# MingruiYuan/SpoofSV

Hardware: AMD Instinct MI355X
Metric: mel-frames/sec (Text2Mel+SSRN train) (higher is better)
Workload: dtype f32 (conv GEMMs: fp32 operands scaled by a power of two and split into fp16 hi+lo = 22 significand bits, three exact fp16 MFMAs per product, fp32 accumulate: ~2^-22 per product, gradients within 3e-6 of float64 = the exact-fp32 path's level); 1 GPU; train_text2mel + train_ssrn (train/ordinary.py step: fwd, l1+bin-div+guided-att losses, bwd, Adam), batch 32 utterances/GPU, N=186, T=325, 80 mel -> 513x1300 linear, hidden 256, random-init; global_batch=32, parallelism=dp1, launch=hipGraph replay, ddp=none

## Files before the change

spoofsv_amd/csrc/ssv_common.h:

```cpp
#pragma once
#include <hip/hip_runtime.h>
#include <stdint.h>
#include <stddef.h>
#include "../../include/ssv_hip.h"

int ssv_fail(int code, const char* fmt, ...);
#define SSV_BAD_SHAPE (-1)
#define SSV_UNSUPPORTED (-2)
#define SSV_CHECK(cond, code, ...) do { if (!(cond)) return ssv_fail((code), __VA_ARGS__); } while (0)
#define SSV_TRY(expr) do { int _e = (expr); if (_e) return _e; } while (0)
int ssv_check_launch(const char* what);

typedef __attribute__((ext_vector_type(4))) float f32x4;

struct GemmNN {
  const float* A = nullptr; long sab = 0, sam = 0, sac = 0, saj = 0;
  const float* X = nullptr; long sxb = 0, sxc = 0, sxn = 1; int Lx = 0;
  float* C = nullptr; long scb = 0, scm = 0, scn = 1;
  const float* bias = nullptr;
  const float* bias_b = nullptr; long sbb = 0;
  const float* R = nullptr; long srb = 0, srm = 0, srn = 1;
  int M = 0, N = 0, Kc = 0, KT = 1, B = 1;
  int shift[3] = {0, 0, 0};
  float alpha = 1.f;
};
int ssv_launch_gemm_nn(const GemmNN& g, hipStream_t st);

struct GemmNT {
  const float* A = nullptr; long sab = 0, sam = 0, sat = 1; int La = 0;
  const float* X = nullptr; long sxb = 0, sxc = 0, sxn = 1; int Lx = 0;
  float* C = nullptr; long scz = 0, scm = 0, scc = 1, scj = 0;
  int M = 0, Nc = 0, KT = 1, B = 1, Z = 1, bstep = 1;
  int shift[3] = {0, 0, 0};
  const ssv_wgrad_job* jobs = nullptr; int njobs = 0;
  int max_shift = -1;
  int f16 = 0; const float* a_amax = nullptr; int a_namax = 0; const float* x_amax = nullptr; int x_namax = 0;
};
int ssv_launch_gemm_nt(const GemmNT& g, hipStream_t st);

struct GemmNNB {
  const unsigned short* Ahi = nullptr; const unsigned short* Alo = nullptr; int Kpad = 0;
  const float* X = nullptr; long sxb = 0, sxc = 0; int Lx = 0;
  float* C = nullptr; long scb = 0, scm = 0;
  const float* bias = nullptr;
  const float* bias_b = nullptr; long sbb = 0;
  const float* R = nullptr; long srb = 0, srm = 0;
  int M = 0, N = 0, Kc = 0, KT = 1, B = 1;
  int shift[3] = {0, 0, 0};
  int sxn = 1, scn = 1;
  int row_pair = 0; float* c_amax = nullptr; int c_namax = 0;
  unsigned short* hs_planes = nullptr; long hs_plane_bytes = 0; int hs_npad = 0;
  int hs_keep_h = 1;
  int ksplit = 1; long scz = 0; int skip_rows = 0;
  const unsigned short* x0_planes = nullptr; const float* x0_amax = nullptr; int xsplit0 = 0;
  int perm_h = 0, epi = 0, first = 0;
  float* cstate = nullptr;
  float* lstm_out = nullptr; int lstm_s = 0, lstm_lo = 0, lstm_D = 0, xsplit = 0; long sab = 0;
  const unsigned short* A0hi = nullptr; const unsigned short* A0lo = nullptr;
  float* gates_out = nullptr;
  int f16 = 0; const float* a_inv = nullptr; const float* x_amax = nullptr; int x_namax = 0; long x_amax_bs = 0;
  float* colstats = nullptr;
  const float* xrow_w = nullptr; long xrow_sk = 0;
};
int ssv_launch_gemm_nn_bf3(const GemmNNB& g, hipStream_t st);
int ssv_launch_gemm_pwln(const GemmNNB& g, const float* gamma, const float* beta, float* y, long ybs, float* stats, float* y_amax, int namax, int act,
                         hipStream_t st);
int ssv_launch_gemm_nt_bf3(const GemmNT& g, hipStream_t st);
int ssv_launch_gemm_nt3r(const GemmNT& g, dim3 grid, int mtiles, int tchunks, int ring_ms, hipStream_t st);
struct PwLnBw {
  const float* dy; long dy_bs; const float* pre; const float* stats; const float* gamma; const float* beta;
  float* dpre; float* part; int part_rows; int part_q; float* amax; int namax;
  const unsigned short* Ahi; const unsigned short* Alo; const float* a_inv;
  float* dx; long dx_bs; const float* xrow_w; long xrow_sk;
  int M, Cin, L, act;
};
bool ssv_pwln_bwd_fused_ok(int B, int Cin, int Cout, int L);
int ssv_launch_pwln_bwd(const PwLnBw& q, int B, int f16, hipStream_t st);
bool ssv_nt_bf3_xrow(int KT, int M, int Nc);
bool ssv_nt_bf3_fits(const GemmNT& g);
int ssv_launch_pack_split(const float* w, void* hi, void* lo, int M, int K, int Kpad, int KT, long sm, long sk, long sj, int perm_h, hipStream_t st,
                          int nch_total = 0, int ch_off = 0);
int ssv_launch_pack_split_f16(const float* w, long w_elems, void* hi, void* lo, int M, int K, int Kpad, int KT, long sm, long sk, long sj, float* aux, hipStream_t st);
int ssv_launch_pack_split_f16_list(const float* w, void* hi, void* lo, int M, int K, int Kpad, int KT, long sm, long sk, long sj, int perm_h,
                                   const float* list, int nlist, float* inv_out, hipStream_t st, int nch_total = 0, int ch_off = 0);
#define SSV_F16_AUX_FLOATS 128
#define SSV_AMAX_FALLBACK 64
int ssv_launch_absmax(const float* x, long x_bs, int B, long n, float* out, int npb, hipStream_t st);
int ssv_nt_bf3_tiles(int KT, int M, int Nc);
void ssv_nt_bf3_tile(int KT, int M, int Nc, int* wm, int* ntc);
int ssv_nt_bf3_wg_per_cu(int KT, int wm, int ntc);
int ssv_precision();
enum { SSV_T_NT_FORCE, SSV_T_NNB_FORCE, SSV_T_LN_GROUPS, SSV_T_LN_PERSIST, SSV_T_LSTM_MERGE, SSV_T_PWLN_BWD, SSV_T_COUNT };
const char* ssv_tuning(int knob);
int ssv_pack_job_blocks(const ssv_pack_job& j);
int ssv_launch_pack_multi(const ssv_pack_job* jobs_dev, int njobs, int nblocks, float* amax_ws, hipStream_t st);
#define SSV_PACK_AMAX_PER_WEIGHT 32

int ssv_launch_reduce_slabs(const float* slabs, float* out, long n, int Z, long slab_stride, hipStream_t st);
int ssv_launch_reduce_slabs_perm(const float* slabs, float* out, int M, int Nc, int KT, int Z, hipStream_t st);
int ssv_launch_reduce_pair(const float* slabs, float* out, int M, int Nc, int KT, int Z, const float* part, float* pout, int n2, int nblk, hipStream_t st);
int ssv_launch_reduce_pair_multi(const ssv_wgrad_job* jobs, int njobs, const float* slabs, int M, int Nc, int KT, int Z, int n2, int nblk, hipStream_t st);
int ssv_launch_pack_wt(const float* w, float* wt, int Cout, int Cin, int KT, hipStream_t st);
int ssv_launch_fill(float* p, float v, long n, hipStream_t st);
int ssv_launch_linear_len1_fwd(const float* x, long x_bs, const float* w, const float* bias, const float* bias_b, long sbb, float* y, long y_bs,
                               int B, int K, int M, hipStream_t st);
int ssv_launch_linear_len1_wgrad(const float* dy, long dy_bs, const float* x, long x_bs, float* dw, int B, int K, int M, hipStream_t st);

static inline int ssv_cdiv(long a, long b) { return (int)((a + b - 1) / b); }
bool ssv_shape_log_on();
void ssv_shape_log(const char* kernel, dim3 grid, dim3 block, double flops, double bytes, const char* note);
__host__ __device__ static inline int ssv_amax_rows_(int L) { return 4 * ((L + 63) / 64); }

__device__ __forceinline__ unsigned ssv_xcd_order(unsigned lin, unsigned total) {
  const unsigned xcd = lin & 7u, idx = lin >> 3, q = total >> 3, r = total & 7u;
  return xcd * q + (xcd < r ? xcd : r) + idx;
}

__device__ __forceinline__ void ssv_pow2_scale(float amax, float& scale, float& inv) {
  int E = (int)((__float_as_uint(amax) >> 23) & 0xffu);
  E = min(max(E, 15), 254);
  scale = __uint_as_float((unsigned)(268 - E) << 23);
  inv = __uint_as_float((unsigned)(E - 14) << 23);
}
typedef unsigned ssv_u32x4g __attribute__((vector_size(16)));
__device__ __forceinline__ __amdgpu_buffer_rsrc_t ssv_buf(const void* base) {
  return __builtin_amdgcn_make_buffer_rsrc(const_cast<void*>(base), 0, -1, 0x00020000);
}
__device__ __forceinline__ float ssv_buf_f32(__amdgpu_buffer_rsrc_t r, unsigned voff, unsigned soff) {
  return __builtin_bit_cast(float, __builtin_amdgcn_raw_buffer_load_b32(r, (int)voff, (int)soff, 0));
}
__device__ __forceinline__ uint4 ssv_buf_u4(__amdgpu_buffer_rsrc_t r, unsigned voff, unsigned soff) {
  return __builtin_bit_cast(uint4, __builtin_amdgcn_raw_buffer_load_b128(r, (int)voff, (int)soff, 0));
}
template <class T> __device__ __forceinline__ T* ssv_global(T* p) {
  return (T*)(__attribute__((address_space(1))) T*)p;
}
__device__ __forceinline__ float ssv_uniform(float v) { return __builtin_bit_cast(float, __builtin_amdgcn_readfirstlane(__builtin_bit_cast(int, v))); }
template <int NW>
__device__ __forceinline__ float ssv_wg_max(float v, float* sm) {
#pragma unroll
  for (int o = 1; o < 64; o <<= 1) v = fmaxf(v, __shfl_xor(v, o));
  if ((threadIdx.x & 63) == 0) sm[threadIdx.x >> 6] = v;
  __syncthreads();
  float r = sm[0];
#pragma unroll
  for (int i = 1; i < NW; ++i) r = fmaxf(r, sm[i]);
  return r;
}
template <int CTRL> __device__ __forceinline__ float ssv_dpp_mov(float v);
template <int CTRL>
__device__ __forceinline__ float ssv_dpp_max(float v) { return fmaxf(v, ssv_dpp_mov<CTRL>(v)); }
__device__ __forceinline__ float ssv_wave_list_max(const float* __restrict__ p, int n) {
  float v = 0.f;
  for (int i = threadIdx.x & 63; i < n; i += 64) v = fmaxf(v, p[i]);
  v = ssv_dpp_max<0xB1>(v);
  v = ssv_dpp_max<0x4E>(v);
  v = ssv_dpp_max<0x141>(v);
  v = ssv_dpp_max<0x140>(v);
  const int b = __builtin_bit_cast(int, v);
  const float r0 = __builtin_bit_cast(float, __builtin_amdgcn_readlane(b, 0)), r1 = __builtin_bit_cast(float, __builtin_amdgcn_readlane(b, 16));
  const float r2 = __builtin_bit_cast(float, __builtin_amdgcn_readlane(b, 32)), r3 = __builtin_bit_cast(float, __builtin_amdgcn_readlane(b, 48));
  return fmaxf(fmaxf(r0, r1), fmaxf(r2, r3));
}
template <int NW>
__device__ __forceinline__ float ssv_list_max(const float* __restrict__ p, int n, float* sm) {
  float v = 0.f;
  for (int i = threadIdx.x; i < n; i += 64 * NW) v = fmaxf(v, p[i]);
  return ssv_wg_max<NW>(v, sm);
}

template <int CTRL>
__device__ __forceinline__ float ssv_dpp_mov(float v) {
  return __builtin_bit_cast(float, __builtin_amdgcn_update_dpp(0, __builtin_bit_cast(int, v), CTRL, 0xf, 0xf, true));
}
__device__ __forceinline__ float ssv_row16_sum(float v) {
  v += ssv_dpp_mov<0xB1>(v);
  v += ssv_dpp_mov<0x4E>(v);
  v += ssv_dpp_mov<0x141>(v);
  v += ssv_dpp_mov<0x140>(v);
  return v;
}
__device__ __forceinline__ float ssv_wave_sum(float v) {
  v = ssv_row16_sum(v);
  v += __shfl_xor(v, 16);
  v += __shfl_xor(v, 32);
  return v;
}
```

spoofsv_amd/csrc/wgrad_nt.hip:

```cpp
#include "bf3_common.h"

#ifdef SSV_NT_STAMP
__device__ unsigned long long ssv_nt_stamps[64];
__device__ unsigned long long ssv_nt_wg[4096 * 4];
extern "C" int ssv_debug_nt_wg(unsigned long long* out) { return (int)hipMemcpyFromSymbol(out, HIP_SYMBOL(ssv_nt_wg), sizeof(ssv_nt_wg)); }
#define NT_WG(k, v) do { const unsigned w_ = blockIdx.z * gridDim.x + blockIdx.x; if (threadIdx.x == 0 && w_ < 4096u) ssv_nt_wg[w_ * 4 + (k)] = (v); } while (0)
#define NT_STAMP(k) do { if (stamp_on && (unsigned)(stamp_s - 24) < 8u) ssv_nt_stamps[(stamp_s - 24) * 8 + (k)] = __builtin_readcyclecounter(); } while (0)
extern "C" int ssv_debug_nt_stamps(unsigned long long* out) { return (int)hipMemcpyFromSymbol(out, HIP_SYMBOL(ssv_nt_stamps), sizeof(ssv_nt_stamps)); }
#else
#define NT_STAMP(k) do {} while (0)
#define NT_WG(k, v) do {} while (0)
#endif
constexpr int NT_FD = 1;
template <int KT, int WM, int NTC, int F16, int XR = 0, int WV = 4>
__global__ __launch_bounds__(64 * WV, WV == 4 ? 2 : 1) void gemm_nt_bf3_kernel(const GemmNT p, const int mtiles) {
  constexpr int NTH = 64 * WV;
  constexpr int KB = 64, KG = KB / 8, KS = KB / 32;
  constexpr int NCH = 16 * NTC;
  constexpr int X_SLOTS = KG * NCH;
  constexpr int NX = X_SLOTS / NTH;
  static_assert(X_SLOTS % NTH == 0, "tile slots must be a multiple of the workgroup size");
  __shared__ uint4 lds[2][2 * X_SLOTS];
  __shared__ float amax_sm[2 * WV];

  const int tid = threadIdx.x, lane = tid & 63, wave = tid >> 6;
  NT_WG(0, __builtin_amdgcn_s_memrealtime()); NT_WG(2, __builtin_readcyclecounter());
  const unsigned wg = ssv_xcd_order(blockIdx.x + gridDim.x * blockIdx.z, gridDim.x * gridDim.z);
  const int bxx = (int)(wg % gridDim.x);
  int z = (int)(wg / gridDim.x);
  const float* __restrict__ Ap = p.A;
  const float* __restrict__ Xp = p.X;
  float* __restrict__ Cp = p.C;
  int shj[3] = {p.shift[0], p.shift[1], p.shift[2]};
  const float* __restrict__ a_amax = p.a_amax;
  const float* __restrict__ x_amax = p.x_amax;
  int a_namax = p.a_namax, x_namax = p.x_namax;
  if (p.jobs) {
    const int job = z / p.Z;
    z -= job * p.Z;
    const ssv_wgrad_job* __restrict__ jb = p.jobs + job;
    Ap = ssv_global(jb->dy); Xp = ssv_global(jb->x); Cp = p.C + (long)job * p.Z * p.scz;
    shj[0] = jb->shift[0]; shj[1] = jb->shift[1]; shj[2] = jb->shift[2];
    a_amax = ssv_global(jb->dy_amax); x_amax = ssv_global(jb->x_amax); a_namax = jb->dy_namax; x_namax = jb->x_namax;
  }
  float as = 1.f, xs = 1.f, us = 1.f;
  auto scales = [&]() {
    if constexpr (F16) {
      float sa, sx, ia, ix;
      ssv_pow2_scale(ssv_list_max<WV>(a_amax, a_namax, amax_sm), sa, ia);
      ssv_pow2_scale(ssv_list_max<WV>(x_amax, x_namax, amax_sm + WV), sx, ix);
      as = ssv_uniform(sa); xs = ssv_uniform(sx);
      us = ssv_uniform(ia * ix);
    }
  };
  const int ctiles_ = (int)gridDim.x / mtiles;
  const bool ct_fast = gridDim.x > 64u;
  const int mt = ct_fast ? bxx / ctiles_ : bxx % mtiles, ct = ct_fast ? bxx % ctiles_ : bxx / mtiles;
  const int m0 = mt * 16 * WV * WM, c0 = ct * NCH;
  const int tchunks = (p.La + KB - 1) / KB;
  const int kq = lane >> 4, nq = lane & 15;

  f32x4 acc[WM][KT][NTC];
#pragma unroll
  for (int i = 0; i < WM; ++i)
#pragma unroll
    for (int j = 0; j < KT; ++j)
#pragma unroll
      for (int q = 0; q < NTC; ++q) acc[i][j][q] = (f32x4){0.f, 0.f, 0.f, 0.f};

  float rx[NX][8];
  int mx[NX];
  static_assert(!XR || (KT == 1 && WV == 4 && (256 % KG) == 0), "extra row: k = 1; a thread's slots share their k-group");
  const bool xr_on = XR && mt == 0;
  float xacc[XR ? NX : 1];
  uint4 xra[XR ? 2 : 1];
#pragma unroll
  for (int r = 0; r < (XR ? NX : 1); ++r) xacc[r] = 0.f;
  uint4 AH[2][WM][KS], AL[2][WM][KS];

  const __amdgpu_buffer_rsrc_t rsA = __builtin_amdgcn_make_buffer_rsrc(const_cast<float*>(Ap), 0,
      (int)(((long)(p.B - 1) * p.sab + (long)(p.M - 1) * p.sam + p.La) * 4), 0x00020000);
  const int x_span = (int)((long)(p.B - 1) * p.sxb + (long)(p.Nc - 1) * p.sxc + p.Lx) - 8;
  int arow[WM], xrow[NX];
#pragma unroll
  for (int i = 0; i < WM; ++i) arow[i] = (min(m0 + wave * WM * 16 + i * 16 + nq, p.M - 1) * (int)p.sam + 8 * kq) * 4;
  const int xra_off = ((p.M - 1) * (int)p.sam + 8 * (tid % KG)) * 4;
#pragma unroll
  for (int r = 0; r < NX; ++r) {
    const int f = tid + NTH * r;
    xrow[r] = min(c0 + f / KG, p.Nc - 1) * (int)p.sxc + 8 * (f % KG);
  }
  const bool rows_in_c = c0 + NCH <= p.Nc;

  auto load8 = [&](const float* __restrict__ base, int off, float (&v)[8]) {
    typedef __attribute__((address_space(1))) const char gchar;
    typedef __attribute__((address_space(1))) const f4u gf4u;
    gchar* q = (gchar*)reinterpret_cast<const char*>(base) + ((unsigned)off << 2);
    const f4u a = *(gf4u*)q;
    const f4u c = *(gf4u*)(q + 16);
    v[0] = a.x; v[1] = a.y; v[2] = a.z; v[3] = a.w; v[4] = c.x; v[5] = c.y; v[6] = c.z; v[7] = c.w;
  };
  auto load8c = [&](const float* __restrict__ base, int off, int span, float (&v)[8]) -> int {
    const int oc = min(max(off, 0), span);
    load8(base, oc, v);
    return off - oc;
  };
  auto edge_meta = [&](int d, int t, int len, bool row_ok, int over2 = 0) -> int {
    const int sl = min(max(-t, 0), 8), sh = max(min(max(t + 8 - len, 0), 8), min(max(over2, 0), 8));
    const int m = row_ok ? (int)((0xFFu << sl) & (0xFFu >> sh) & 0xFFu) : 0;
    return m | (d << 8);
  };
  auto edge_vals = [&](const float (&raw)[8], int meta, float (&v)[8]) {
#pragma unroll
    for (int i = 0; i < 8; ++i) v[i] = raw[i];
    const int d = meta >> 8;
    if (__builtin_expect(__builtin_amdgcn_ballot_w64(d != 0) != 0ull, 0)) {
#pragma unroll
      for (int i = 0; i < 8; ++i) {
        float r = 0.f;
#pragma unroll
        for (int k = 0; k < 8; ++k) r = (i + d == k) ? raw[k] : r;
        v[i] = r;
      }
    }
#pragma unroll
    for (int i = 0; i < 8; ++i) v[i] = ((meta >> i) & 1) ? v[i] : 0.f;
  };
  auto split_edge = [&](const float (&raw)[8], int meta, float sc, uint4& h, uint4& l) {
    float v[8];
    edge_vals(raw, meta, v);
    split8p<F16>(v, sc, h, l);
  };

  const int bstep = p.bstep > 0 ? p.bstep : 1;
  int total, cb[4], ct0[4];
  if (p.bstep > 0) {
    total = ((p.B - z + p.bstep - 1) / p.bstep) * tchunks;
    cb[0] = z; ct0[0] = 0;
  } else {
    const int all = p.B * tchunks, per = (all + p.Z - 1) / p.Z, start = z * per;
    total = max(min(per, all - start), 0);
    cb[0] = start / tchunks; ct0[0] = (start % tchunks) * KB;
  }
  auto next_chunk = [&](int b, int t0, int& nb_, int& nt0) __attribute__((always_inline)) {
    nt0 = t0 + KB; nb_ = b;
    if (nt0 >= tchunks * KB) { nt0 = 0; nb_ = b + bstep; }
  };
#pragma unroll
  for (int k = 1; k < 4; ++k) next_chunk(cb[k - 1], ct0[k - 1], cb[k], ct0[k]);
  auto x_edge = [&](int t0, int j) __attribute__((always_inline)) -> bool {
    return !(rows_in_c && t0 + shj[j] >= 0 && t0 + KB + shj[j] <= p.Lx && t0 + KB <= p.La);
  };

  auto loadA = [&](auto set, int b, int t0) __attribute__((always_inline)) {
    constexpr int SET = decltype(set)::value;
    const unsigned so = (unsigned)(b * (int)p.sab + t0) * 4u;
#pragma unroll
    for (int i = 0; i < WM; ++i)
#pragma unroll
      for (int s2 = 0; s2 < KS; ++s2) {
        AH[SET][i][s2] = __builtin_bit_cast(uint4, __builtin_amdgcn_raw_buffer_load_b128(rsA, arow[i] + s2 * 128, (int)so, 0));
        AL[SET][i][s2] = __builtin_bit_cast(uint4, __builtin_amdgcn_raw_buffer_load_b128(rsA, arow[i] + s2 * 128 + 16, (int)so, 0));
      }
  };
  auto raw8 = [&](const uint4& t0_, const uint4& t1_, float (&v)[8]) __attribute__((always_inline)) {
    v[0] = __builtin_bit_cast(float, t0_.x); v[1] = __builtin_bit_cast(float, t0_.y); v[2] = __builtin_bit_cast(float, t0_.z); v[3] = __builtin_bit_cast(float, t0_.w);
    v[4] = __builtin_bit_cast(float, t1_.x); v[5] = __builtin_bit_cast(float, t1_.y); v[6] = __builtin_bit_cast(float, t1_.z); v[7] = __builtin_bit_cast(float, t1_.w);
  };
  auto splitA = [&](auto set) __attribute__((always_inline)) {
    constexpr int SET = decltype(set)::value;
#pragma unroll
    for (int i = 0; i < WM; ++i)
#pragma unroll
      for (int s2 = 0; s2 < KS; ++s2) {
        float v[8];
        raw8(AH[SET][i][s2], AL[SET][i][s2], v);
        split8p<F16>(v, as, AH[SET][i][s2], AL[SET][i][s2]);
      }
  };
  auto loadX = [&](int b, int t0, int j) __attribute__((always_inline)) {
    const int base = b * (int)p.sxb + t0 + shj[j];
    int dd[NX];
#pragma unroll
    for (int r = 0; r < NX; ++r) dd[r] = load8c(Xp, base + xrow[r], x_span, rx[r]);
    if constexpr (XR) {
      const unsigned so = (unsigned)(b * (int)p.sab + t0) * 4u;
      xra[0] = __builtin_bit_cast(uint4, __builtin_amdgcn_raw_buffer_load_b128(rsA, xra_off, (int)so, 0));
      xra[1] = __builtin_bit_cast(uint4, __builtin_amdgcn_raw_buffer_load_b128(rsA, xra_off + 16, (int)so, 0));
    }
    if (x_edge(t0, j)) {
#pragma unroll
      for (int r = 0; r < NX; ++r) {
        const int f = tid + NTH * r;
        mx[r] = edge_meta(dd[r], t0 + shj[j] + 8 * (f % KG), p.Lx, c0 + f / KG < p.Nc, t0 + 8 * (f % KG) + 8 - p.La);
      }
    }
  };
  auto commitX = [&](auto buf, int t0, int j) __attribute__((always_inline)) {
    constexpr int S = decltype(buf)::value;
    uint4* Xh = lds[S];
    uint4* Xl = lds[S] + X_SLOTS;
    const bool edge = x_edge(t0, j);
#pragma unroll
    for (int r = 0; r < NX; ++r) {
      const int f = tid + NTH * r;
      const int kg = f % KG, c = f / KG;
      uint4 h, l;
      if (!edge) split8p<F16>(rx[r], xs, h, l);
      else split_edge(rx[r], mx[r], xs, h, l);
      Xh[kg * NCH + (c ^ kg)] = h; Xl[kg * NCH + (c ^ kg)] = l;
      if constexpr (XR) {
        if (xr_on) {
          float av[8], xv[8];
          raw8(xra[0], xra[1], av);
          if (!edge) {
#pragma unroll
            for (int i = 0; i < 8; ++i) xv[i] = rx[r][i];
          } else edge_vals(rx[r], mx[r], xv);
#pragma unroll
          for (int i = 0; i < 8; ++i) xacc[r] = __builtin_fmaf(av[i], xv[i], xacc[r]);
        }
      }
    }
  };
  using P0 = std::integral_constant<int, 0>;
  using P1 = std::integral_constant<int, 1>;
  const int steps = total * KT;

  auto chunk = [&](auto steady, auto par, int n) __attribute__((always_inline)) {
    constexpr bool STEADY = decltype(steady)::value;
    constexpr int PAR = decltype(par)::value;
    const bool more = STEADY || n + 1 < total;
#ifdef SSV_NT_STAMP
    const bool stamp_on = blockIdx.x == 0 && blockIdx.z == 0 && tid == 0;
#endif
    using CUR = std::integral_constant<int, PAR>;
    using NXT = std::integral_constant<int, PAR ^ 1>;
    if (more) loadA(NXT{}, cb[1], ct0[1]);
#pragma unroll
    for (int j = 0; j < KT; ++j) {
      const int q_ = (PAR + j) & 1;
#ifdef SSV_NT_STAMP
      const int stamp_s = n * KT + j;
#endif
      NT_STAMP(0);
      const uint4* Xh = lds[q_];
      const uint4* Xl = lds[q_] + X_SLOTS;
      constexpr int G = KS * NTC;
      uint4 fb[NT_FD + 1][2];
      auto frag = [&](int g, uint4 (&f)[2]) __attribute__((always_inline)) {
        const int kg = (g / NTC) * 4 + kq;
        const int xs_ = kg * NCH + (((g % NTC) * 16 + nq) ^ kg);
        f[0] = Xh[xs_]; f[1] = Xl[xs_];
      };
#pragma unroll
      for (int g = 0; g < NT_FD; ++g) frag(g, fb[g]);
#pragma unroll
      for (int g = 0; g < G; ++g) {
        if (g + NT_FD < G) frag(g + NT_FD, fb[(g + NT_FD) % (NT_FD + 1)]);
        __builtin_amdgcn_sched_barrier(0);
        const int s2 = g / NTC, q = g % NTC;
        const uint4 bh = fb[g % (NT_FD + 1)][0];
        const uint4 bl = fb[g % (NT_FD + 1)][1];
#pragma unroll
        for (int i = 0; i < WM; ++i) {
          const uint4 a_h = AH[CUR::value][i][s2];
          const uint4 a_l = AL[CUR::value][i][s2];
          acc[i][j][q] = mma16<F16>(a_l, bh, acc[i][j][q]);
          acc[i][j][q] = mma16<F16>(a_h, bl, acc[i][j][q]);
          acc[i][j][q] = mma16<F16>(a_h, bh, acc[i][j][q]);
        }
      }
      NT_STAMP(1);
      const int c1 = (j + 1) / KT, j1 = (j + 1) % KT;
      const int c2 = (j + 2) / KT, j2 = (j + 2) % KT;
      const int s = n * KT + j;
#ifdef SSV_NT_STAMP
      asm volatile("" : "+v"(rx[NX - 1][7]));
      NT_STAMP(6);
#endif
      if (STEADY || s + 1 < steps) {
        if (((PAR + j) & 1) == 0) commitX(P1{}, ct0[c1], j1); else commitX(P0{}, ct0[c1], j1);
      }
      NT_STAMP(2);
      if (j == KT - 1 && more) splitA(NXT{});
      NT_STAMP(3);
      if (STEADY || s + 2 < steps) loadX(cb[c2], ct0[c2], j2);
      NT_STAMP(4);
      __syncthreads();
      NT_STAMP(5);
    }
#pragma unroll
    for (int k = 0; k < 3; ++k) { cb[k] = cb[k + 1]; ct0[k] = ct0[k + 1]; }
    next_chunk(cb[2], ct0[2], cb[3], ct0[3]);
  };

  if (total > 0) {
    loadA(P0{}, cb[0], ct0[0]);
    loadX(cb[0], ct0[0], 0);
    scales();
    splitA(P0{});
    commitX(P0{}, ct0[0], 0);
    if (steps > 1) loadX(cb[1 / KT], ct0[1 / KT], 1 % KT);
    __syncthreads();
    using ST = std::integral_constant<bool, true>;
    using TL = std::integral_constant<bool, false>;
    const int nfull = (steps - 2) / KT;
    static_assert((KT & 1) == 1, "chunk parities alternate");
    int n = 0;
    for (; n + 1 < nfull; n += 2) {
      chunk(ST{}, P0{}, n);
      chunk(ST{}, P1{}, n + 1);
    }
    for (; n < total; n += 2) {
      chunk(TL{}, P0{}, n);
      if (n + 1 < total) chunk(TL{}, P1{}, n + 1);
    }
  }

  NT_WG(3, __builtin_readcyclecounter());
  float* __restrict__ Cz = Cp + (long)z * p.scz;
#pragma unroll
  for (int i = 0; i < WM; ++i)
#pragma unroll
    for (int r = 0; r < 4; ++r) {
      const int gm = m0 + wave * WM * 16 + i * 16 + kq * 4 + r;
      if (gm >= (XR ? p.M - 1 : p.M)) continue;
#pragma unroll
      for (int j = 0; j < KT; ++j)
#pragma unroll
        for (int q = 0; q < NTC; ++q) {
          const int gc = c0 + q * 16 + nq;
          if (gc < p.Nc) Cz[(long)gm * p.scm + (long)gc * p.scc + (long)j * p.scj] = F16 ? acc[i][j][q][r] * us : acc[i][j][q][r];
        }
    }
  if constexpr (XR) {
    if (xr_on) {
#pragma unroll
      for (int r = 0; r < NX; ++r) {
        float v = xacc[r];
        v += __shfl_xor(v, 1); v += __shfl_xor(v, 2); v += __shfl_xor(v, 4);
        const int f = tid + NTH * r, gc = c0 + f / KG;
        if ((f % KG) == 0 && gc < p.Nc) Cz[(long)(p.M - 1) * p.scm + (long)gc * p.scc] = v;
      }
    }
  }
#ifdef SSV_NT_STAMP
  __builtin_amdgcn_s_waitcnt(0);
#endif
  NT_WG(1, __builtin_amdgcn_s_memrealtime());
}

void ssv_nt_bf3_tile(int KT, int M, int Nc, int* wm, int* ntc) {
  if (KT == 3) { *wm = 2; *ntc = 4; }
  else if (Nc <= 48) { *wm = 2; *ntc = 2; }
  else if (M % 256 == 0 && Nc % 128 == 0 && (long)M * Nc >= (1L << 21)) { *wm = 4; *ntc = 8; }
  else if (M % 128 == 0 && Nc % 128 == 0 && (long)M * Nc >= (1L << 21)) { *wm = 2; *ntc = 8; }
  else if ((long)M * Nc >= (1L << 18)) { *wm = 2; *ntc = 6; }
  else { *wm = 1; *ntc = 4; }
}
int ssv_nt_bf3_wg_per_cu(int KT, int wm, int ntc) {
  if (wm == 4) return 1;
  if (KT == 3) return wm == 2 ? 2 : (ntc >= 4 ? 3 : 4);
  if (wm == 2) return ntc >= 6 ? 2 : 3;
  return ntc >= 6 ? 3 : (ntc >= 4 ? 4 : 5);
}
int ssv_nt_bf3_tiles(int KT, int M, int Nc) {
  int wm, ntc;
  ssv_nt_bf3_tile(KT, M, Nc, &wm, &ntc);
  return ssv_cdiv(ssv_nt_bf3_xrow(KT, M, Nc) ? M - 1 : M, 64 * wm) * ssv_cdiv(Nc, 16 * ntc);
}
bool ssv_nt_bf3_xrow(int KT, int M, int Nc) {
  int wm, ntc;
  ssv_nt_bf3_tile(KT, M, Nc, &wm, &ntc);
  return KT == 1 && wm == 2 && ntc == 6 && M > 128 && M % 128 == 1;
}

bool ssv_nt_bf3_fits(const GemmNT& g) {
  const long lim = 1L << 30;
  return (long)(g.B - 1) * g.sab + (long)(g.M - 1) * g.sam + g.La < lim && (long)(g.B - 1) * g.sxb + (long)(g.Nc - 1) * g.sxc + g.Lx < lim &&
         (long)g.B * g.sab < lim && (long)g.B * g.sxb < lim && g.La >= 8 && g.Lx >= 8;
}
int ssv_launch_gemm_nt_bf3(const GemmNT& g, hipStream_t st) {
  SSV_CHECK(g.M > 0 && g.Nc > 0 && g.La > 0 && g.B > 0 && g.Z > 0 && g.bstep >= 0, SSV_BAD_SHAPE, "gemm_nt_bf3: empty problem");
  SSV_CHECK(g.KT == 1 || g.KT == 3, SSV_UNSUPPORTED, "gemm_nt_bf3: kernel_size %d", g.KT);
  SSV_CHECK(g.sat == 1 && g.sxn == 1, SSV_UNSUPPORTED, "gemm_nt_bf3: rows must be contiguous in time");
  SSV_CHECK(g.Z <= 65535, SSV_UNSUPPORTED, "gemm_nt_bf3: Z=%d exceeds grid.z", g.Z);
  SSV_CHECK(ssv_nt_bf3_fits(g), SSV_UNSUPPORTED, "gemm_nt_bf3: an operand spans 2^30 elements or more");
  int wm, ntc;
  ssv_nt_bf3_tile(g.KT, g.M, g.Nc, &wm, &ntc);
  const bool xr = ssv_nt_bf3_xrow(g.KT, g.M, g.Nc);
  SSV_CHECK(g.bstep > 0 || xr, SSV_UNSUPPORTED, "gemm_nt_bf3: range slabs are built for the extra-row kernel only");
  const int mtiles = ssv_cdiv(xr ? g.M - 1 : g.M, 64 * wm);
  const int nz = g.jobs ? g.njobs * g.Z : g.Z;
  SSV_CHECK(nz <= 65535, SSV_UNSUPPORTED, "gemm_nt_bf3: %d slabs exceed grid.z", nz);
  const dim3 grid(mtiles * ssv_cdiv(g.Nc, 16 * ntc), 1, nz);
  SSV_CHECK(!g.f16 || g.jobs || (g.a_amax && g.x_amax && g.a_namax > 0 && g.x_namax > 0), SSV_BAD_SHAPE, "gemm_nt_bf3: split-fp16 needs both operand scales");
  int ring_ms = -1;
  if (g.KT == 3 && wm == 2 && ntc == 4) {
    ring_ms = g.max_shift;
    if (!g.jobs) { ring_ms = 0; for (int j = 0; j < 3; ++j) ring_ms = abs(g.shift[j]) > ring_ms ? abs(g.shift[j]) : ring_ms; }
    if (ring_ms > 64) ring_ms = -1;
  }
  if (ssv_shape_log_on()) {
    char nm[96], note[96];
    const int nj = g.jobs ? g.njobs : 1;
    if (ring_ms >= 0) snprintf(nm, sizeof nm, "gemm_nt3r_kernel<%d, %d>", wm, g.f16);
    else if (wm == 4) snprintf(nm, sizeof nm, "gemm_nt_bf3_kernel<%d, 2, %d, %d, 0, 8>", g.KT, ntc, g.f16);
    else snprintf(nm, sizeof nm, "gemm_nt_bf3_kernel<%d, %d, %d, %d, %d, 4>", g.KT, wm, ntc, g.f16, xr ? 1 : 0);
    snprintf(note, sizeof note, "jobs=%d B=%d M=%d Nc=%d L=%d k=%d Z=%d", nj, g.B, g.M, g.Nc, g.La, g.KT, g.Z);
    ssv_shape_log(nm, grid, dim3(wm == 4 ? 512 : 256), 2.0 * nj * g.B * g.M * g.Nc * g.La * g.KT,
                  4.0 * nj * ((double)g.B * g.M * g.La + (double)g.B * g.Nc * g.Lx + (double)g.Z * g.M * g.Nc * g.KT), note);
  }
  if (ring_ms >= 0) {
    const int tchunks = ssv_cdiv((g.La > g.Lx ? g.La : g.Lx) + ring_ms, 64);
    return ssv_launch_gemm_nt3r(g, grid, mtiles, tchunks, ring_ms, st);
  }
  if (xr) {
    if (g.f16) hipLaunchKernelGGL((gemm_nt_bf3_kernel<1, 2, 6, 1, 1>), grid, dim3(256), 0, st, g, mtiles);
    else hipLaunchKernelGGL((gemm_nt_bf3_kernel<1, 2, 6, 0, 1>), grid, dim3(256), 0, st, g, mtiles);
    return ssv_check_launch("gemm_nt_bf3 (extra row)");
  }
  if (g.KT == 1 && wm == 4 && ntc == 8) {
    if (g.f16) hipLaunchKernelGGL((gemm_nt_bf3_kernel<1, 2, 8, 1, 0, 8>), grid, dim3(512), 0, st, g, mtiles);
    else hipLaunchKernelGGL((gemm_nt_bf3_kernel<1, 2, 8, 0, 0, 8>), grid, dim3(512), 0, st, g, mtiles);
    return ssv_check_launch("gemm_nt_bf3 (8 waves)");
  }
#define SSV_NT(K_, A_, C_) if (g.KT == K_ && wm == A_ && ntc == C_) { \
    if (g.f16) hipLaunchKernelGGL((gemm_nt_bf3_kernel<K_, A_, C_, 1>), grid, dim3(256), 0, st, g, mtiles); \
    else hipLaunchKernelGGL((gemm_nt_bf3_kernel<K_, A_, C_, 0>), grid, dim3(256), 0, st, g, mtiles); \
    return ssv_check_launch("gemm_nt_bf3"); }
  SSV_NT(3, 2, 4)
  SSV_NT(1, 2, 8) SSV_NT(1, 2, 6) SSV_NT(1, 2, 2) SSV_NT(1, 1, 4)
#undef SSV_NT
  return ssv_fail(SSV_UNSUPPORTED, "gemm_nt_bf3: no tile %d,%d for kernel size %d", wm, ntc, g.KT);
}
```

spoofsv_amd/csrc/wgrad_nt3r.hip:

```cpp
#include "bf3_common.h"

#ifdef SSV_NT_STAMP
__device__ unsigned long long ssv_nt3r_stamps[64];
__device__ unsigned long long ssv_nt3r_wg[4096 * 4];
extern "C" int ssv_debug_nt3r_wg(unsigned long long* out) { return (int)hipMemcpyFromSymbol(out, HIP_SYMBOL(ssv_nt3r_wg), sizeof(ssv_nt3r_wg)); }
extern "C" int ssv_debug_nt3r_stamps(unsigned long long* out) { return (int)hipMemcpyFromSymbol(out, HIP_SYMBOL(ssv_nt3r_stamps), sizeof(ssv_nt3r_stamps)); }
#define NT_WG(k, v) do { const unsigned w_ = blockIdx.z * gridDim.x + blockIdx.x; if (threadIdx.x == 0 && w_ < 4096u) ssv_nt3r_wg[w_ * 4 + (k)] = (v); } while (0)
#define NT_STAMP(k) do { if (stamp_on && (unsigned)(stamp_s - 24) < 8u) ssv_nt3r_stamps[(stamp_s - 24) * 8 + (k)] = __builtin_readcyclecounter(); } while (0)
#else
#define NT_STAMP(k) do {} while (0)
#define NT_WG(k, v) do {} while (0)
#endif
typedef short ssv_s4 __attribute__((ext_vector_type(4)));
typedef __attribute__((address_space(3))) ssv_s4 ssv_lds_s4;
typedef unsigned ssv_u2 __attribute__((ext_vector_type(2)));
typedef __attribute__((address_space(3))) ssv_u2 ssv_lds_u2;
__device__ __forceinline__ void ssv_lds_store2(unsigned addr, unsigned a, unsigned b) {
#if defined(__HIP_DEVICE_COMPILE__)
  *(ssv_lds_u2*)(size_t)addr = (ssv_u2){a, b};
#else
  (void)addr; (void)a; (void)b;
#endif
}
__device__ __forceinline__ uint2 ssv_lds_read_tr16(unsigned addr) {
#if defined(__HIP_DEVICE_COMPILE__)
  return __builtin_bit_cast(uint2, __builtin_amdgcn_ds_read_tr16_b64_v4i16((ssv_lds_s4*)(size_t)addr));
#else
  (void)addr; return make_uint2(0u, 0u);
#endif
}
template <int WM, int F16>
__global__ __launch_bounds__(256, 2) void gemm_nt3r_kernel(const GemmNT p, const int mtiles, const int tchunks, const int max_shift) {
  constexpr int KT = 3, NTC = 4, NCH = 64, KB = 64, KS = 2;
  constexpr int R_FD = 1;
  constexpr unsigned ROWB = 128, PLANE = 288 * ROWB;
  __shared__ __attribute__((aligned(16))) unsigned char ring[2 * PLANE];
  __shared__ float amax_sm[8];

  const int tid = threadIdx.x, lane = tid & 63, wave = tid >> 6;
  NT_WG(0, __builtin_amdgcn_s_memrealtime()); NT_WG(2, __builtin_readcyclecounter());
  const unsigned wg = ssv_xcd_order(blockIdx.x + gridDim.x * blockIdx.z, gridDim.x * gridDim.z);
  const int bxx = (int)(wg % gridDim.x);
  int z = (int)(wg / gridDim.x);
  const float* __restrict__ Ap = p.A;
  const float* __restrict__ Xp = p.X;
  float* __restrict__ Cp = p.C;
  int shj[3] = {p.shift[0], p.shift[1], p.shift[2]};
  const float* __restrict__ a_amax = p.a_amax;
  const float* __restrict__ x_amax = p.x_amax;
  int a_namax = p.a_namax, x_namax = p.x_namax;
  if (p.jobs) {
    const int job = z / p.Z;
    z -= job * p.Z;
    const ssv_wgrad_job* __restrict__ jb = p.jobs + job;
    Ap = ssv_global(jb->dy); Xp = ssv_global(jb->x); Cp = p.C + (long)job * p.Z * p.scz;
    shj[0] = jb->shift[0]; shj[1] = jb->shift[1]; shj[2] = jb->shift[2];
    a_amax = ssv_global(jb->dy_amax); x_amax = ssv_global(jb->x_amax); a_namax = jb->dy_namax; x_namax = jb->x_namax;
  }
  float as = 1.f, xs = 1.f, us = 1.f;
  if constexpr (F16) {
    float sa, sx, ia, ix;
    ssv_pow2_scale(ssv_list_max<4>(a_amax, a_namax, amax_sm), sa, ia);
    ssv_pow2_scale(ssv_list_max<4>(x_amax, x_namax, amax_sm + 4), sx, ix);
    as = ssv_uniform(sa); xs = ssv_uniform(sx);
    us = ssv_uniform(ia * ix);
  }
  const int mt = bxx % mtiles, ct = bxx / mtiles;
  const int m0 = mt * 64 * WM, c0 = ct * NCH;
  const int kq = lane >> 4, nq = lane & 15;

  f32x4 acc[WM][KT][NTC];
#pragma unroll
  for (int i = 0; i < WM; ++i)
#pragma unroll
    for (int j = 0; j < KT; ++j)
#pragma unroll
      for (int q = 0; q < NTC; ++q) acc[i][j][q] = (f32x4){0.f, 0.f, 0.f, 0.f};

  uint4 AH[2][WM][KS], AL[2][WM][KS];
  uint4 rx[4];

  const __amdgpu_buffer_rsrc_t rsA = __builtin_amdgcn_make_buffer_rsrc(const_cast<float*>(Ap), 0,
      (int)(((long)(p.B - 1) * p.sab + (long)(p.M - 1) * p.sam + p.La) * 4), 0x00020000);
  const __amdgpu_buffer_rsrc_t rsX = __builtin_amdgcn_make_buffer_rsrc(const_cast<float*>(Xp), 0,
      (int)(((long)(p.B - 1) * p.sxb + (long)(p.Nc - 1) * p.sxc + p.Lx) * 4), 0x00020000);
  const unsigned arow = (unsigned)(((m0 + wave * WM * 16 + nq) * (int)p.sam + 4 * kq) * 4);
  const unsigned a16 = 16u * (unsigned)p.sam * 4u;
  const int cq = lane >> 4, tq = lane & 15;
  const unsigned xrow = (unsigned)(((c0 + 16 * wave + 4 * cq) * (int)p.sxc + 4 * tq) * 4);
  const unsigned x1 = (unsigned)p.sxc * 4u;
  const bool rows_in_c = c0 + NCH <= p.Nc;
  const unsigned ringb = (unsigned)(size_t)(__attribute__((address_space(3))) unsigned char*)ring;
  const unsigned waddr = ringb + (unsigned)(4 * tq) * ROWB + (unsigned)((wave ^ ((tq & 1) | (((tq >> 2) & 1) << 1))) << 5) + (unsigned)cq * 8u;
  const int q4 = (lane >> 2) & 3, pp = lane & 3;
  int lrow[2];
  lrow[0] = 4 * kq + (q4 >> 1) + 16 * (q4 & 1);
  lrow[1] = lrow[0] + 2;
  unsigned lbase[2], key5[KT][2];
#pragma unroll
  for (int r = 0; r < 2; ++r) {
    lbase[r] = ringb + (unsigned)lrow[r] * ROWB + (unsigned)pp * 8u;
#pragma unroll
    for (int j = 0; j < KT; ++j) { const int rr = shj[j] + lrow[r]; key5[j][r] = (unsigned)(((rr >> 2) & 1) | (((rr >> 4) & 1) << 1)) << 5; }
  }

  const int nb = (p.B - z + p.bstep - 1) / p.bstep;
  const int total = nb * tchunks;
  int cb[4], ct0[4];
  cb[0] = z; ct0[0] = 0;
  auto next_chunk = [&](int b, int t0, int& nb_, int& nt0) __attribute__((always_inline)) {
    nt0 = t0 + KB; nb_ = b;
    if (nt0 >= tchunks * KB) { nt0 = 0; nb_ = b + p.bstep; }
  };
#pragma unroll
  for (int k = 1; k < 4; ++k) next_chunk(cb[k - 1], ct0[k - 1], cb[k], ct0[k]);

  auto loadA = [&](auto set, int b, int t0) __attribute__((always_inline)) {
    constexpr int SET = decltype(set)::value;
    const unsigned so = ((unsigned)b * (unsigned)p.sab + (unsigned)t0) * 4u;
#pragma unroll
    for (int i = 0; i < WM; ++i)
#pragma unroll
      for (int s2 = 0; s2 < KS; ++s2) {
        AH[SET][i][s2] = __builtin_bit_cast(uint4, __builtin_amdgcn_raw_buffer_load_b128(rsA, (int)(arow + (so + i * a16)) + s2 * 128, 0, 0));
        AL[SET][i][s2] = __builtin_bit_cast(uint4, __builtin_amdgcn_raw_buffer_load_b128(rsA, (int)(arow + (so + i * a16)) + s2 * 128 + 64, 0, 0));
      }
  };
  auto loadA1 = [&](auto set, int b, int t0, int idx) __attribute__((always_inline)) {
    constexpr int SET = decltype(set)::value;
    const unsigned so = ((unsigned)b * (unsigned)p.sab + (unsigned)t0) * 4u;
    const int i = idx / (2 * KS), s2 = (idx / 2) % KS, hf = idx % 2;
    const uint4 v = __builtin_bit_cast(uint4, __builtin_amdgcn_raw_buffer_load_b128(rsA, (int)(arow + (so + i * a16)) + s2 * 128 + 64 * hf, 0, 0));
    if (hf) AL[SET][i][s2] = v; else AH[SET][i][s2] = v;
  };
  auto loadX1 = [&](int b, int t0, int ci) __attribute__((always_inline)) {
    const unsigned so = ((unsigned)b * (unsigned)p.sxb + (unsigned)t0) * 4u;
    rx[ci] = __builtin_bit_cast(uint4, __builtin_amdgcn_raw_buffer_load_b128(rsX, (int)(xrow + (so + ci * x1)), 0, 0));
  };
  auto splitA = [&](auto set, int t0) __attribute__((always_inline)) {
    constexpr int SET = decltype(set)::value;
    const bool ragged = t0 + KB > p.La;
#pragma unroll
    for (int i = 0; i < WM; ++i)
#pragma unroll
      for (int s2 = 0; s2 < KS; ++s2) {
        float v[8];
        const uint4 t0_ = AH[SET][i][s2], t1_ = AL[SET][i][s2];
        v[0] = __builtin_bit_cast(float, t0_.x); v[1] = __builtin_bit_cast(float, t0_.y); v[2] = __builtin_bit_cast(float, t0_.z); v[3] = __builtin_bit_cast(float, t0_.w);
        v[4] = __builtin_bit_cast(float, t1_.x); v[5] = __builtin_bit_cast(float, t1_.y); v[6] = __builtin_bit_cast(float, t1_.z); v[7] = __builtin_bit_cast(float, t1_.w);
        if (ragged) {
          const int nv = p.La - (t0 + 32 * s2 + 4 * kq);
#pragma unroll
          for (int e = 0; e < 8; ++e) v[e] = (e >= 4 ? e + 12 : e) < nv ? v[e] : 0.f;
        }
        split8p<F16>(v, as, AH[SET][i][s2], AL[SET][i][s2]);
      }
  };
  auto loadX = [&](int b, int t0) __attribute__((always_inline)) {
    const unsigned so = ((unsigned)b * (unsigned)p.sxb + (unsigned)t0) * 4u;
#pragma unroll
    for (int ci = 0; ci < 4; ++ci) rx[ci] = __builtin_bit_cast(uint4, __builtin_amdgcn_raw_buffer_load_b128(rsX, (int)(xrow + (so + ci * x1)), 0, 0));
  };
  auto commitX = [&](int slot, int t0) __attribute__((always_inline)) {
    float v[4][4];
#pragma unroll
    for (int ci = 0; ci < 4; ++ci) {
      v[ci][0] = __builtin_bit_cast(float, rx[ci].x); v[ci][1] = __builtin_bit_cast(float, rx[ci].y);
      v[ci][2] = __builtin_bit_cast(float, rx[ci].z); v[ci][3] = __builtin_bit_cast(float, rx[ci].w);
    }
    if (!(rows_in_c && t0 + KB <= p.Lx)) {
      const int nv = p.Lx - (t0 + 4 * tq);
#pragma unroll
      for (int ci = 0; ci < 4; ++ci) {
        const bool cok = c0 + 16 * wave + 4 * cq + ci < p.Nc;
#pragma unroll
        for (int i = 0; i < 4; ++i) v[ci][i] = (cok && i < nv) ? v[ci][i] : 0.f;
      }
    }
    const unsigned a = waddr + (unsigned)slot * (64u * ROWB);
#pragma unroll
    for (int i = 0; i < 4; ++i) {
      unsigned h0, l0, h1, l1;
      split_pair<F16>(v[0][i], v[1][i], xs, h0, l0);
      split_pair<F16>(v[2][i], v[3][i], xs, h1, l1);
      ssv_lds_store2(a + i * ROWB, h0, h1);
      ssv_lds_store2(a + i * ROWB + PLANE, l0, l1);
      if (slot == 0 && tq < 8) {
        ssv_lds_store2(a + i * ROWB + 256u * ROWB, h0, h1);
        ssv_lds_store2(a + i * ROWB + 256u * ROWB + PLANE, l0, l1);
      }
    }
  };
  using P0 = std::integral_constant<int, 0>;
  using P1 = std::integral_constant<int, 1>;

  auto chunk = [&](auto par, int n) __attribute__((always_inline)) {
    using CUR = std::integral_constant<int, decltype(par)::value>;
    using NXT = std::integral_constant<int, decltype(par)::value ^ 1>;
#ifdef SSV_NT_STAMP
    const bool stamp_on = blockIdx.x == 0 && blockIdx.z == 0 && tid == 0;
    const int stamp_s = n + 16;
#endif
    NT_STAMP(0);
#pragma unroll
    for (int j = 0; j < KT; ++j) {
      constexpr int G = KS * NTC;
      uint4 fb[R_FD + 1][2];
      unsigned su[KS];
#pragma unroll
      for (int s2 = 0; s2 < KS; ++s2) su[s2] = (unsigned)((64 * n + shj[j] + 32 * s2) & 255) * ROWB;
      auto frag = [&](int g, uint4 (&f)[2]) __attribute__((always_inline)) {
        const int s2 = g / NTC, cbk = g % NTC;
        const unsigned a0 = lbase[0] + su[s2] + ((unsigned)(cbk << 5) ^ key5[j][0]);
        const unsigned a1 = lbase[1] + su[s2] + ((unsigned)(cbk << 5) ^ key5[j][1]);
        const uint2 h0u = ssv_lds_read_tr16(a0), h1u = ssv_lds_read_tr16(a1);
        const uint2 l0u = ssv_lds_read_tr16(a0 + PLANE), l1u = ssv_lds_read_tr16(a1 + PLANE);
        f[0] = make_uint4(h0u.x, h0u.y, h1u.x, h1u.y);
        f[1] = make_uint4(l0u.x, l0u.y, l1u.x, l1u.y);
      };
#pragma unroll
      for (int g = 0; g < R_FD; ++g) frag(g, fb[g]);
#pragma unroll
      for (int g = 0; g < G; ++g) {
        if (g + R_FD < G) frag(g + R_FD, fb[(g + R_FD) % (R_FD + 1)]);
        if (j == 0 && g < 4 * WM) loadA1(NXT{}, cb[1], ct0[1], g);
        if (j == 1 && g < 4) loadX1(cb[3], ct0[3], g);
        __builtin_amdgcn_sched_barrier(0);
        const int s2 = g / NTC, q = g % NTC;
        if (ct0[0] + 32 * s2 >= p.La) continue;
        const uint4 bh = fb[g % (R_FD + 1)][0];
        const uint4 bl = fb[g % (R_FD + 1)][1];
#pragma unroll
        for (int i = 0; i < WM; ++i) {
          const uint4 a_h = AH[CUR::value][i][s2];
          const uint4 a_l = AL[CUR::value][i][s2];
          acc[i][j][q] = mma16<F16>(a_l, bh, acc[i][j][q]);
          acc[i][j][q] = mma16<F16>(a_h, bl, acc[i][j][q]);
          acc[i][j][q] = mma16<F16>(a_h, bh, acc[i][j][q]);
        }
      }
      if (j == 0) {
        NT_STAMP(2);
        commitX((n + 2) & 3, ct0[2]);
        NT_STAMP(3);
      }
      if (j == 1) NT_STAMP(5);
      if (j == KT - 1) {
        NT_STAMP(6);
        splitA(NXT{}, ct0[1]);
        NT_STAMP(7);
      }
    }
    __syncthreads();
#pragma unroll
    for (int k = 0; k < 3; ++k) { cb[k] = cb[k + 1]; ct0[k] = ct0[k + 1]; }
    next_chunk(cb[2], ct0[2], cb[3], ct0[3]);
  };

  if (total > 0) {
    loadA(P0{}, cb[0], ct0[0]);
    loadX(cb[0], ct0[0]);
    {
#pragma unroll
      for (int i = 0; i < 4; ++i) {
        ssv_lds_store2(waddr + 3u * 64u * ROWB + i * ROWB, 0u, 0u);
        ssv_lds_store2(waddr + 3u * 64u * ROWB + i * ROWB + PLANE, 0u, 0u);
      }
    }
    commitX(0, ct0[0]);
    loadX(cb[1], ct0[1]);
    splitA(P0{}, ct0[0]);
    commitX(1, ct0[1]);
    loadX(cb[2], ct0[2]);
    __syncthreads();
    int n = 0;
    for (; n + 1 < total; n += 2) {
      chunk(P0{}, n);
      chunk(P1{}, n + 1);
    }
    if (n < total) chunk(P0{}, n);
  }

  NT_WG(3, __builtin_readcyclecounter());
  const bool bad_shift = abs(shj[0]) > max_shift || abs(shj[1]) > max_shift || abs(shj[2]) > max_shift;
  float* __restrict__ Cz = Cp + (long)z * p.scz;
#pragma unroll
  for (int i = 0; i < WM; ++i)
#pragma unroll
    for (int r = 0; r < 4; ++r) {
      const int gm = m0 + wave * WM * 16 + i * 16 + kq * 4 + r;
      if (gm >= p.M) continue;
#pragma unroll
      for (int j = 0; j < KT; ++j)
#pragma unroll
        for (int q = 0; q < NTC; ++q) {
          const int gc = c0 + q * 16 + nq;
          if (gc < p.Nc) Cz[(long)gm * p.scm + (long)gc * p.scc + (long)j * p.scj] = bad_shift ? __builtin_nanf("") : (F16 ? acc[i][j][q][r] * us : acc[i][j][q][r]);
        }
    }
#ifdef SSV_NT_STAMP
  __builtin_amdgcn_s_waitcnt(0);
#endif
  NT_WG(1, __builtin_amdgcn_s_memrealtime());
}


int ssv_launch_gemm_nt3r(const GemmNT& g, dim3 grid, int mtiles, int tchunks, int ring_ms, hipStream_t st) {
  if (g.f16) hipLaunchKernelGGL((gemm_nt3r_kernel<2, 1>), grid, dim3(256), 0, st, g, mtiles, tchunks, ring_ms);
  else hipLaunchKernelGGL((gemm_nt3r_kernel<2, 0>), grid, dim3(256), 0, st, g, mtiles, tchunks, ring_ms);
  return ssv_check_launch("gemm_nt3r");
}
```

Baseline: 851,900 mel-frames/s.

## Fuse amax reductions, defer scale computation past prologue loads, trim per-job chunk count

Computes the two per-operand amax reductions in one pass with unrolled buffer loads and a single workgroup barrier, replacing two sequential reductions. In the nt3r kernel the scale computation moves after the first A/X global loads are issued, so the amax latency overlaps with the prologue loads. Each wgrad job also computes its own time-chunk count from its actual shift instead of the launch-wide maximum, which skips empty chunks. Moving the scales after loadA is only safe if loadA does not use them; tchunks per job changes the loop bounds, which risks correctness if a shift is misclassified.

```diff
diff --git a/spoofsv_amd/csrc/ssv_common.h b/spoofsv_amd/csrc/ssv_common.h
--- a/spoofsv_amd/csrc/ssv_common.h
+++ b/spoofsv_amd/csrc/ssv_common.h
@@ -168,6 +168,44 @@
   for (int i = threadIdx.x; i < n; i += 64 * NW) v = fmaxf(v, p[i]);
   return ssv_wg_max<NW>(v, sm);
 }
+template <int NW>
+__device__ __forceinline__ void ssv_list_max2_part(const float* __restrict__ pa, int na, const float* __restrict__ px, int nx, float* sm) {
+  constexpr int U = 4;
+  const __amdgpu_buffer_rsrc_t ra = __builtin_amdgcn_make_buffer_rsrc(const_cast<float*>(pa), 0, na * 4, 0x00020000);
+  const __amdgpu_buffer_rsrc_t rx = __builtin_amdgcn_make_buffer_rsrc(const_cast<float*>(px), 0, nx * 4, 0x00020000);
+  const int nmax = na > nx ? na : nx;
+  float va = 0.f, vx = 0.f;
+  for (int i0 = 0; i0 < nmax; i0 += 64 * NW * U) {
+    float ta[U], tx[U];
+#pragma unroll
+    for (int u = 0; u < U; ++u) ta[u] = ssv_buf_f32(ra, (unsigned)(i0 + (int)threadIdx.x + 64 * NW * u) * 4u, 0u);
+#pragma unroll
+    for (int u = 0; u < U; ++u) tx[u] = ssv_buf_f32(rx, (unsigned)(i0 + (int)threadIdx.x + 64 * NW * u) * 4u, 0u);
+#pragma unroll
+    for (int u = 0; u < U; ++u) { va = fmaxf(va, ta[u]); vx = fmaxf(vx, tx[u]); }
+  }
+  float v[2] = {va, vx};
+#pragma unroll
+  for (int k = 0; k < 2; ++k) {
+    float t = v[k];
+    t = ssv_dpp_max<0xB1>(t);
+    t = ssv_dpp_max<0x4E>(t);
+    t = ssv_dpp_max<0x141>(t);
+    t = ssv_dpp_max<0x140>(t);
+    const int b = __builtin_bit_cast(int, t);
+    const float r0 = __builtin_bit_cast(float, __builtin_amdgcn_readlane(b, 0)), r1 = __builtin_bit_cast(float, __builtin_amdgcn_readlane(b, 16));
+    const float r2 = __builtin_bit_cast(float, __builtin_amdgcn_readlane(b, 32)), r3 = __builtin_bit_cast(float, __builtin_amdgcn_readlane(b, 48));
+    v[k] = fmaxf(fmaxf(r0, r1), fmaxf(r2, r3));
+  }
+  if ((threadIdx.x & 63) == 0) { sm[threadIdx.x >> 6] = v[0]; sm[NW + (threadIdx.x >> 6)] = v[1]; }
+}
+template <int NW>
+__device__ __forceinline__ void ssv_list_max2_read(const float* sm, float& amax_a, float& amax_x) {
+  float a = sm[0], x = sm[NW];
+#pragma unroll
+  for (int i = 1; i < NW; ++i) { a = fmaxf(a, sm[i]); x = fmaxf(x, sm[NW + i]); }
+  amax_a = a; amax_x = x;
+}
 
 template <int CTRL>
 __device__ __forceinline__ float ssv_dpp_mov(float v) {
diff --git a/spoofsv_amd/csrc/wgrad_nt.hip b/spoofsv_amd/csrc/wgrad_nt.hip
--- a/spoofsv_amd/csrc/wgrad_nt.hip
+++ b/spoofsv_amd/csrc/wgrad_nt.hip
@@ -46,9 +46,12 @@
   float as = 1.f, xs = 1.f, us = 1.f;
   auto scales = [&]() {
     if constexpr (F16) {
-      float sa, sx, ia, ix;
-      ssv_pow2_scale(ssv_list_max<WV>(a_amax, a_namax, amax_sm), sa, ia);
-      ssv_pow2_scale(ssv_list_max<WV>(x_amax, x_namax, amax_sm + WV), sx, ix);
+      float m_a, m_x, sa, sx, ia, ix;
+      ssv_list_max2_part<WV>(a_amax, a_namax, x_amax, x_namax, amax_sm);
+      __syncthreads();
+      ssv_list_max2_read<WV>(amax_sm, m_a, m_x);
+      ssv_pow2_scale(m_a, sa, ia);
+      ssv_pow2_scale(m_x, sx, ix);
       as = ssv_uniform(sa); xs = ssv_uniform(sx);
       us = ssv_uniform(ia * ix);
     }
diff --git a/spoofsv_amd/csrc/wgrad_nt3r.hip b/spoofsv_amd/csrc/wgrad_nt3r.hip
--- a/spoofsv_amd/csrc/wgrad_nt3r.hip
+++ b/spoofsv_amd/csrc/wgrad_nt3r.hip
@@ -30,7 +30,7 @@
 #endif
 }
 template <int WM, int F16>
-__global__ __launch_bounds__(256, 2) void gemm_nt3r_kernel(const GemmNT p, const int mtiles, const int tchunks, const int max_shift) {
+__global__ __launch_bounds__(256, 2) void gemm_nt3r_kernel(const GemmNT p, const int mtiles, const int tchunks_launch, const int max_shift) {
   constexpr int KT = 3, NTC = 4, NCH = 64, KB = 64, KS = 2;
   constexpr int R_FD = 1;
   constexpr unsigned ROWB = 128, PLANE = 288 * ROWB;
@@ -57,14 +57,12 @@
     shj[0] = jb->shift[0]; shj[1] = jb->shift[1]; shj[2] = jb->shift[2];
     a_amax = ssv_global(jb->dy_amax); x_amax = ssv_global(jb->x_amax); a_namax = jb->dy_namax; x_namax = jb->x_namax;
   }
+  int tchunks = tchunks_launch;
+  if (p.jobs) {
+    const int own_shift = max(max(abs(shj[0]), abs(shj[1])), abs(shj[2]));
+    if (own_shift <= max_shift) tchunks = ((p.La > p.Lx ? p.La : p.Lx) + own_shift + KB - 1) / KB;
+  }
   float as = 1.f, xs = 1.f, us = 1.f;
-  if constexpr (F16) {
-    float sa, sx, ia, ix;
-    ssv_pow2_scale(ssv_list_max<4>(a_amax, a_namax, amax_sm), sa, ia);
-    ssv_pow2_scale(ssv_list_max<4>(x_amax, x_namax, amax_sm + 4), sx, ix);
-    as = ssv_uniform(sa); xs = ssv_uniform(sx);
-    us = ssv_uniform(ia * ix);
-  }
   const int mt = bxx % mtiles, ct = bxx / mtiles;
   const int m0 = mt * 64 * WM, c0 = ct * NCH;
   const int kq = lane >> 4, nq = lane & 15;
@@ -267,6 +265,16 @@
         ssv_lds_store2(waddr + 3u * 64u * ROWB + i * ROWB + PLANE, 0u, 0u);
       }
     }
+    if constexpr (F16) {
+      ssv_list_max2_part<4>(a_amax, a_namax, x_amax, x_namax, amax_sm);
+      __syncthreads();
+      float m_a, m_x, sa, sx, ia, ix;
+      ssv_list_max2_read<4>(amax_sm, m_a, m_x);
+      ssv_pow2_scale(m_a, sa, ia);
+      ssv_pow2_scale(m_x, sx, ix);
+      as = ssv_uniform(sa); xs = ssv_uniform(sx);
+      us = ssv_uniform(ia * ix);
+    }
     commitX(0, ct0[0]);
     loadX(cb[1], ct0[1]);
     splitA(P0{}, ct0[0]);
```

Result: no change. 857,500 mel-frames/s, median of 6 (+0.7%).
